# huakunyang/SummerTTS

Measured on AMD Instinct MI355X. Metric: audio samples/sec (acoustic model + vocoder, phoneme ids -> int16 PCM on host), single_speaker_fast-shaped synthetic blob, higher is better.
Workload: dtype f32 (decoder trunk convs AND the reverse flow's WaveNet convs (wn_flow.hip, one-utterance calls): fp32 operands as 2 fp16 terms = 22-23 of their 24 mantissa bits, 3 fp16 MFMA products per fp32 product, f32 accumulation -- measured error in `parity`, same tolerance as the exact-fp32 leg; batches addi

## Files before the change

include/summertts_hip.h:

```cpp
#ifndef SUMMERTTS_HIP_H_
#define SUMMERTTS_HIP_H_

#include <stdint.h>

#ifdef __cplusplus
extern "C" {
#endif

typedef struct sts_engine sts_engine;

enum {
    STS_OK = 0,
    STS_EINVAL = -1,
    STS_EMODEL = -2,
    STS_EDEVICE = -3,
    STS_ESTATE = -4
};

int sts_create(const float* blob, int64_t blob_bytes, int device, sts_engine** out);
void sts_destroy(sts_engine* e);

int sts_speaker_num(const sts_engine* e);

typedef struct sts_model_info {
// ... 100 lines not shown
#define STS_EQ_MAX_BANDS 4
#define STS_EQ_PEAK 1
#define STS_EQ_LOWSHELF 2
#define STS_EQ_HIGHSHELF 3
#define STS_EQ_HIGHPASS 4
#define STS_EQ_LOWPASS 5
typedef struct sts_eq_band { int32_t type; float freq_hz; float gain_db; float q; } sts_eq_band;
int sts_set_eq(sts_engine* e, int32_t n_bands, const sts_eq_band* bands);
int sts_get_eq(const sts_engine* e, int32_t* n_bands, sts_eq_band* bands, int32_t capacity);
int sts_eq_check(int32_t rate, int32_t n_bands, const sts_eq_band* bands);
int sts_eq_design(int32_t rate, int32_t n_bands, const sts_eq_band* bands, double* coeffs);
int sts_eq_apply(int device, const float* x, const int64_t* lengths, int32_t B, int32_t rate, int32_t n_bands,
                 const sts_eq_band* bands, float* y, int16_t* pcm);
int sts_set_record_taps(sts_engine* e, int enable);
int sts_get_tap(sts_engine* e, const char* name, float** data, int32_t* channels, int64_t* length);
int sts_get_durations(sts_engine* e, int32_t* dur, int64_t capacity);
int sts_set_conv_mode(sts_engine* e, int mode);
int sts_set_conv_math(sts_engine* e, int mode);

enum { STS_DBG_ATTN_BLOCK_MIN_WGS = 1,
       STS_DBG_TAIL_FUSED = 14 ,
       STS_DBG_UPS_ROWPH = 15 ,
       STS_DBG_CHAIN_STREAMS = 13 ,
       STS_DBG_H2P = 11 ,
       STS_DBG_H2P_TILE = 12 ,
       STS_DBG_MEMO_CLEAR = 10 ,
       STS_DBG_PCM_DIRECT = 9 ,
       STS_DBG_DDS_TAIL = 8 ,
       STS_DBG_ATTN_REG = 7 ,
       STS_DBG_LAUNCH_AHEAD = 6 ,
       STS_DBG_FLOW_FUSED = 5  };
enum { STS_DBG_STREAM_RETRY_STEP = 16, STS_DBG_STREAM_DIRECT = 17 };
enum { STS_DBG_POISON = 18 };
int sts_debug_set(sts_engine* e, int key, int value);

typedef struct sts_profile {
    float ms_text_encoder, ms_duration, ms_flow, ms_decoder, ms_total_device;
    float ms_decoder_mfma;
    int32_t decoder_mfma_launches;
    double flops_text_encoder, flops_duration, flops_flow, flops_decoder;
    double flops_decoder_mfma;
    double bytes_decoder_min;
    int64_t frames, samples, phonemes;
    double flops_decoder_mfma_executed;
    double bytes_text_encoder, bytes_duration, bytes_flow;
    float ms_sync_wait_host;
    double flops_decoder_bf16_issued;
    int64_t conv_math_fallbacks;
    int32_t conv_math_pinned;
    int32_t launch_ahead;
    int64_t launch_ahead_misses;
    float us_host_setup;
    float us_host_enqueue;
    float us_host_tail;
    int64_t poison_bytes;
} sts_profile;
int sts_set_profiling(sts_engine* e, int enable);
#define STS_ABI_VERSION 16
int sts_abi_version(void);
int sts_build_flags(void);
int sts_get_profile(const sts_engine* e, sts_profile* p);
int sts_get_profile_ex(const sts_engine* e, void* p, int64_t size_bytes);

int sts_debug_conv1d(int device, const float* x, int32_t Cin, int32_t L, const float* w, const float* bias,
                     int32_t Cout, int32_t k, int32_t pad, int32_t dil, int32_t stride_transposed,
                     int32_t depthwise, float in_slope, int32_t in_act, int mode, float** y, int32_t* Lout);
// ... 93 lines not shown
```

summertts_amd/csrc/capi.hip:

```cpp
#include <stdlib.h>
#include <string.h>

#include <algorithm>
#include <new>
#include <string>
#include <vector>

#include "engine.hpp"

using namespace sts;

struct sts_engine { Engine eng; };

static thread_local std::string g_err;
static int set_err(int code, const std::string& s) { g_err = s; return code; }

extern "C" {

const char* sts_last_error(void) { return g_err.c_str(); }
void sts_free(void* p) { free(p); }

int sts_create(const float* blob, int64_t blob_bytes, int device, sts_engine** out) {
    if (!out) return set_err(STS_EINVAL, "sts_create: null out pointer");
    *out = nullptr;
// ... 564 lines not shown
    if (!e) return set_err(STS_EINVAL, "null engine");
    if (noise_scale) *noise_scale = e->eng.noise.ns;
    if (noise_scale_w) *noise_scale_w = e->eng.noise.nsw;
    if (seed) *seed = e->eng.noise.seed;
    return STS_OK;
}
int sts_set_record_taps(sts_engine* e, int enable) { if (!e) return set_err(STS_EINVAL, "null engine"); e->eng.record_taps = enable != 0; return STS_OK; }
int sts_set_conv_math(sts_engine* e, int mode) {
    if (!e) return set_err(STS_EINVAL, "null engine");
    if (mode < 0 || mode > 3) return set_err(STS_EINVAL, "conv math: 0 = split-bf16 (default), 1 = exact fp32, 2 = split-bf16 wherever eligible, 3 = two-term fp16");
    e->eng.conv_math = mode;
    e->eng.h2_consecutive = 0; e->eng.h2_disabled = false;
    return STS_OK;
}
int sts_set_conv_mode(sts_engine* e, int mode) { if (!e) return set_err(STS_EINVAL, "null engine"); e->eng.conv_mode = mode; return STS_OK; }
int sts_debug_set(sts_engine* e, int key, int value) {
    if (!e) return set_err(STS_EINVAL, "null engine");
    switch (key) {
        case STS_DBG_ATTN_BLOCK_MIN_WGS: if (value < 1) return set_err(STS_EINVAL, "threshold must be >= 1"); e->eng.attn_block_min_wgs = value; return STS_OK;
        case STS_DBG_FLOW_FUSED: e->eng.flow_fused = value != 0; return STS_OK;
        case STS_DBG_LAUNCH_AHEAD: if (value < 0 || value > 2) return set_err(STS_EINVAL, "launch_ahead must be 0, 1 or 2"); if ((value == 2) != (e->eng.launch_ahead == 2)) { e->eng.seen_tf_.clear(); e->eng.seen_order_.clear(); } e->eng.launch_ahead = value; return STS_OK;
        case STS_DBG_H2P: e->eng.h2p = value < 0 ? 0 : (value > 4 ? 4 : value); return STS_OK;
        case STS_DBG_H2P_TILE: e->eng.h2p_tile = value; return STS_OK;
        case STS_DBG_CHAIN_STREAMS: e->eng.chain_streams_dbg = value; return STS_OK;
        case STS_DBG_TAIL_FUSED: e->eng.tail_fused = value != 0; return STS_OK;
        case STS_DBG_UPS_ROWPH: e->eng.ups_rowph = value != 0; return STS_OK;
        case STS_DBG_MEMO_CLEAR: e->eng.seen_tf_.clear(); e->eng.seen_order_.clear(); return STS_OK;
        case STS_DBG_ATTN_REG: e->eng.attn_reg = value != 0; return STS_OK;
        case STS_DBG_DDS_TAIL: e->eng.dds_tail = value != 0; return STS_OK;
        case STS_DBG_PCM_DIRECT: e->eng.pcm_direct = value != 0; return STS_OK;
        case STS_DBG_STREAM_RETRY_STEP: e->eng.stream_retry_step = value < 0 ? -1 : value; return STS_OK;
        case STS_DBG_STREAM_DIRECT: e->eng.stream_direct = value != 0; return STS_OK;
        case STS_DBG_POISON: e->eng.poison = (unsigned)value; return STS_OK;
        default: return set_err(STS_EINVAL, "unknown debug key");
    }
}
int sts_set_host_pcm(sts_engine* e, int enable) { if (!e) return set_err(STS_EINVAL, "null engine"); e->eng.host_pcm = enable != 0; return STS_OK; }
int sts_set_profiling(sts_engine* e, int enable) { if (!e) return set_err(STS_EINVAL, "null engine"); e->eng.profiling = enable == 2 ? 2 : (enable != 0 ? 1 : 0); return STS_OK; }

int sts_abi_version(void) { return STS_ABI_VERSION; }

int sts_set_output_rate(sts_engine* e, int32_t rate) {
    if (!e) return set_err(STS_EINVAL, "null engine");
    const int rc = e->eng.set_output_rate(rate);
    return rc == STS_OK ? STS_OK : set_err(rc, e->eng.error());
}
int sts_get_output_rate(const sts_engine* e) {
    if (!e) return set_err(STS_EINVAL, "null engine");
    return e->eng.out_rate;
}
int sts_resample_table(int32_t in_rate, int32_t out_rate, int32_t* P, int32_t* Q, int32_t* taps, float* table, int64_t capacity_floats) {
    ResampleDesign d;
    if (!resample_design(in_rate, out_rate, &d)) return set_err(STS_EINVAL, "rates must be integers in [8000, 48000] with P = out / gcd(in, out) <= 1024");
    const int64_t need = (int64_t)d.P * 2 * d.K;
    if (table && capacity_floats < need) return set_err(STS_EINVAL, "table capacity below P * taps floats");
    if (P) *P = d.P;
    if (Q) *Q = d.Q;
    if (taps) *taps = 2 * d.K;
    if (table) resample_table(d, in_rate, out_rate, table);
    return STS_OK;
}
int sts_set_loudness(sts_engine* e, int mode, float target_lufs, float peak_dbfs) {
    if (!e) return set_err(STS_EINVAL, "null engine");
    const int rc = e->eng.set_loudness(mode, target_lufs, peak_dbfs);
    return rc == STS_OK ? STS_OK : set_err(rc, e->eng.error());
}
// ... 631 lines not shown
```

summertts_amd/csrc/decoder.hip:

```cpp
#include "run_ctx.hpp"
#include "knobs.hpp"

#include <math.h>
#include <string.h>
#include <utility>

namespace sts {

static constexpr int MAX_HALO_H2P = 64;

int decoder_halo_frames(const Model& M) {
    double R = M.dec_type == 0 ? (M.conv_post.k - 1) / 2 : (M.conv_post.k - 1) / 2 + 12;
    const int nk = M.n_resk;
    for (int i = M.n_up - 1; i >= 0; i--) {
        double rb = 0;
        for (int j = 0; j < nk; j++) {
            const DResBlock& b = M.rb[(size_t)i * nk + j];
            double r = 0;
            for (size_t d = 0; d < b.c1.size(); d++) r += b.c1[d].dil * (b.c1[d].k - 1) / 2 + b.c2[d].dil * (b.c2[d].k - 1) / 2;
            if (r > rb) rb = r;
        }
        R += rb;
        const DConv& up = M.ups[i];
        R = ceil((R + up.k) / (double)up.stride) + 1;
// ... 48 lines not shown
    StagedMfma
};
static bool is_fused(LayerKind k) { return k == LayerKind::FusedBf3 || k == LayerKind::FusedWino || k == LayerKind::FusedDirect; }

struct LayerArgs {
    ConvGroup G1, G2;
    ResLayerGroup R;
    H2PGroup H1, H2;
    double fl, flw;
};

struct Engine::ResStage {
    Engine& e; const int i, nk, nd0; const DConv& up; const Lvl& l2; const StageBufs b;
    bool grouped = false, per_chain = false, h2p_stage = false;
    int rank[8] = {};
    const float* cur[kMaxGroup] = {};
    ResStage(Engine& e_, int i_, const Lvl& l2_, float* reg, size_t ce)
        : e(e_), i(i_), nk(e_.model.n_resk), nd0(nk > 0 ? (int)e_.model.rb[(size_t)i_ * nk].c1.size() : 0), up(e_.model.ups[i_]), l2(l2_), b{reg, ce, nk} {
        chain_rank(e.model, i, rank);
    }
    const DResBlock& rb(int j) const { return e.model.rb[(size_t)i * nk + j]; }
    hipStream_t aux(int j) const { return e.aux_[rank[j] % kAux]; }
    long fused128_tiles() const { return (long)((l2.max_len + 117) / 118) * l2.nb * nk; }
    void fork() const { (void)hipEventRecord(e.ev_fork_, e.stream); for (int k = 0; k < kAux; k++) (void)hipStreamWaitEvent(e.aux_[k], e.ev_fork_, 0); }
    void join(int n) const { for (int k = 0; k < n; k++) { (void)hipEventRecord(e.ev_join_[k], e.aux_[k]); (void)hipStreamWaitEvent(e.stream, e.ev_join_[k], 0); } }

    bool probe_grouped();
    void plan();
    bool fuse_candidate(int d) const;
    void fill_convs(int d, LayerArgs& A);
    void fill_fused(int d, ResLayerGroup& R) const;
    void fill_h2p(int d, H2PGroup& H1, H2PGroup& H2) const;
    LayerKind plan_layer(int d, LayerArgs& A) const;
    void launch(LayerKind k, int d, const LayerArgs& A) const;
    void book(LayerKind k, const LayerArgs& A);
    void run_grouped(const float** outs);
    void run_forked(const float** outs);
};

bool Engine::ResStage::probe_grouped() {
    ConvGroup G; G.n = nk;
    const double f0 = e.flops_[3], b0 = e.bytes_[3];
    for (int j = 0; j < nk; j++) G.g[j] = e.conv_args(rb(j).c1[0], b.up(), l2, b.up(), l2, ConvOpt(), nullptr);
    e.flops_[3] = f0; e.bytes_[3] = b0;
    return conv_group_eligible(G);
}

void Engine::ResStage::plan() {
    grouped = e.conv_mode == 0 && nk >= 2 && nk <= kMaxGroup;
    for (int j = 0; j < nk && grouped; j++) grouped = (int)rb(j).c1.size() == nd0;
    grouped = grouped && probe_grouped();
    if (!grouped) return;
    static const int chain_streams_env = exp_int("STS_CHAIN_STREAMS", 0);
    const int chain_streams = e.chain_streams_dbg >= 0 ? e.chain_streams_dbg : chain_streams_env;
    per_chain = ((chain_streams >> i) & 1) && nk <= kAux;
    const long h2p_tiles = (long)((l2.max_len + 127) / 128) * (up.Cout / 128) * l2.nb * nk;
    const long h2p_min = up.Cout == 128 ? 768 : 512;
    h2p_stage = e.conv_math == 3 && e.h2p && !per_chain && up.Cout % 128 == 0 && (double)l2.ld * 32.0 < 2.0e9 &&
                (e.h2p == 2 || (e.h2p == 3 && up.Cout == 128) || (e.h2p == 4 && up.Cout != 128) || h2p_tiles >= h2p_min);
    for (int j = 0; j < nk && h2p_stage; j++)
        for (int d = 0; d < nd0 && h2p_stage; d++) {
            const DConv &c1 = rb(j).c1[d], &c2 = rb(j).c2[d];
            h2p_stage = c1.wh2p && c2.wh2p && c1.Cin == up.Cout && c1.Cout == up.Cout && c2.Cin == up.Cout && c2.Cout == up.Cout &&
                        (c1.k & 1) && (c2.k & 1) && c1.dil >= 1 && c2.dil >= 1 && c1.pad == c1.dil * (c1.k - 1) / 2 && c2.pad == c2.dil * (c2.k - 1) / 2 &&
                        c1.dil * (c1.k - 1) <= MAX_HALO_H2P && c2.dil * (c2.k - 1) <= MAX_HALO_H2P && !c1.depthwise && !c2.depthwise && !c1.transposed && !c2.transposed;
        }
}

bool Engine::ResStage::fuse_candidate(int d) const {
// ... 44 lines not shown
    memset(&H1, 0, sizeof(H1)); memset(&H2, 0, sizeof(H2));
    H1.n = H2.n = nk; H1.seg = H2.seg = l2.seg; H1.B = H2.B = l2.nb; H1.max_n = H2.max_n = l2.max_len; H1.ovf = H2.ovf = e.ovf_;
    for (int j = 0; j < nk; j++) {
        const DConv &c1 = rb(j).c1[d], &c2 = rb(j).c2[d];
        float *t1 = b.t1(j), *pn = b.pn(j), *nxt = b.next(j, cur[j]);
        H2PArgs& a1 = H1.g[j];
        a1.xp = d == 0 ? (const void*)b.P0() : (const void*)pn; a1.xp_ld = l2.ld; a1.wb = c1.wh2p; a1.wscale = c1.h2_scale; a1.bias = c1.bias;
        a1.yp = t1; a1.yp_ld = l2.ld; a1.yp_slope = 0.1f;
        a1.Cin = c1.Cin; a1.Cout = c1.Cout; a1.ntap = c1.k; a1.tap_step = c1.dil; a1.tap_off = -c1.pad;
        H2PArgs& a2 = H2.g[j];
        a2.xp = t1; a2.xp_ld = l2.ld; a2.wb = c2.wh2p; a2.wscale = c2.h2_scale; a2.bias = c2.bias;
        a2.res16 = d == 0 ? b.X0() : cur[j]; a2.res_ld = l2.ld;
        if (d + 1 == nd0) { a2.y = nxt; a2.y_ld = l2.ld; }
        else { a2.y16 = nxt; a2.y16_ld = l2.ld; a2.yp = pn; a2.yp_slope = 0.1f; a2.yp_ld = l2.ld; }
        a2.Cin = c2.Cin; a2.Cout = c2.Cout; a2.ntap = c2.k; a2.tap_step = c2.dil; a2.tap_off = -c2.pad;
    }
}

LayerKind Engine::ResStage::plan_layer(int d, LayerArgs& A) const {
    const bool bf3 = e.conv_math != 1;
    if (fuse_candidate(d)) {
        fill_fused(d, A.R);
        if (resblock_layer_eligible(A.R)) {
            if (bf3 && resblock_bf3_eligible(A.R)) return LayerKind::FusedBf3;
            static const bool no_wino = exp_flag("STS_NO_WINO");
            return !no_wino && resblock_wino_eligible(A.R) ? LayerKind::FusedWino : LayerKind::FusedDirect;
        }
    }
    if (h2p_stage) { fill_h2p(d, A.H1, A.H2); return LayerKind::H2PPair; }
    if (per_chain) return bf3 ? LayerKind::StagedBf3 : LayerKind::StagedMfma;
    return bf3 && conv_bf3_group_eligible(A.G1) && conv_bf3_group_eligible(A.G2) ? LayerKind::StagedBf3 : LayerKind::StagedMfma;
}

void Engine::ResStage::launch(LayerKind k, int d, const LayerArgs& A) const {
    const hipStream_t stream = e.stream;
    static const char* gt = exp_env("STS_GROUP_TILE");
    const int gtile = gt && (int)strlen(gt) > i ? gt[i] - '0' : -1;
    if (is_fused(k)) {
        auto run = [&](const ResLayerGroup& R, hipStream_t st) {
            static const int bv = exp_int("STS_BF3_LAYER_VARIANT", -1);
            if (k == LayerKind::FusedBf3) resblock_bf3(R, st, bv);
            else if (k == LayerKind::FusedWino) resblock_wino(R, st);
            else resblock_layer(R, st);
        };
        if (!per_chain) return run(A.R, stream);
        for (int j = 0; j < nk; j++) { ResLayerGroup R1 = A.R; R1.n = 1; R1.g[0] = A.R.g[j]; run(R1, aux(j)); }
    } else if (k == LayerKind::H2PPair) {
        if (d == 0) split_planes(b.up(), l2.ld, up.Cout, l2.seg, l2.nb, l2.max_len, 0.1f, b.P0(), b.X0(), l2.ld, e.ovf_, stream);
        const int ht = e.h2p_tile < 0 ? -1 : (up.Cout == 128 ? (e.h2p_tile & 0xff) : ((e.h2p_tile >> 8) & 0xff));
        conv_h2p_group(A.H1, stream, ht == 0xff ? -1 : ht);
        conv_h2p_group(A.H2, stream, ht == 0xff ? -1 : ht);
    } else if (per_chain) {
        for (int j = 0; j < nk; j++)
            for (const ConvArgs* ca : {&A.G1.g[j], &A.G2.g[j]}) {
                if (k == LayerKind::StagedBf3 && conv_bf3_eligible(*ca)) conv_bf3(*ca, aux(j), -1);
                else if (conv_mfma_eligible(*ca)) conv_mfma(*ca, aux(j), gtile);
                else conv_generic(*ca, aux(j));
            }
    } else if (k == LayerKind::StagedBf3) {
        static const char* bgt = exp_env("STS_BF3_GROUP_TILE");
        const int bt = bgt && (int)strlen(bgt) > i ? (bgt[i] >= '0' && bgt[i] <= '9' ? bgt[i] - '0' : (bgt[i] >= 'a' && bgt[i] <= 'z' ? bgt[i] - 'a' + 10 : -1)) : -1;
        conv_bf3_group(A.G1, stream, bt);
        conv_bf3_group(A.G2, stream, bt);
    } else {
        for (const ConvGroup* G : {&A.G1, &A.G2}) {
            if (conv_group_eligible(*G)) conv_mfma_group(*G, stream, gtile);
            else for (int j = 0; j < nk; j++) { if (conv_mfma_eligible(G->g[j])) conv_mfma(G->g[j], stream, -1); else conv_generic(G->g[j], stream); }
        }
    }
}

void Engine::ResStage::book(LayerKind k, const LayerArgs& A) {
    e.mfma_flops_ += A.fl;
    if (k == LayerKind::FusedWino) e.mfma_exec_ += A.flw;
    else if (k == LayerKind::FusedDirect || k == LayerKind::StagedMfma) e.mfma_exec_ += A.fl;
    else e.bf16_exec_ += e.products() * A.fl;
    e.mfma_launches_ += is_fused(k) ? 1 : 2;
}

void Engine::ResStage::run_grouped(const float** outs) {
    LayerArgs A;
    for (int j = 0; j < nk; j++) cur[j] = b.up();
    if (per_chain) fork();
    for (int d = 0; d < nd0; d++) {
        fill_convs(d, A);
        const LayerKind k = plan_layer(d, A);
        launch(k, d, A);
        book(k, A);
        for (int j = 0; j < nk; j++) cur[j] = b.next(j, cur[j]);
    }
    if (per_chain) join(kAux);
    for (int j = 0; j < nk; j++) outs[j] = cur[j];
}

void Engine::ResStage::run_forked(const float** outs) {
    const bool forked = nk > 1 && nk <= 8;
    if (forked) fork();
    for (int j = 0; j < nk; j++) {
        if (forked) e.cur_ = aux(j);
        const float* x = b.up();
        for (size_t d = 0; d < rb(j).c1.size(); d++) {
            const auto o = resblock_opts(x);
            float* nxt = b.next(j, x);
            e.conv(rb(j).c1[d], x, l2, b.t1(j), l2, o.first);
            e.conv(rb(j).c2[d], b.t1(j), l2, nxt, l2, o.second);
            x = nxt;
        }
        outs[j] = x;
    }
    if (forked) { join(nk < kAux ? nk : kAux); e.cur_ = e.stream; }
}

int Engine::run_decode(RunCtx& c, int nw, long Wtot, int maxW, int zoff0, int wlen0) {
    RUN_ALIASES(c)
    stage_begin(3);
    const WinGeom win{nw == 1 && !no_inline_seg && wlen0 >= 0, nw, zoff0, wlen0, d_win};
    auto lvF = [&](int scale, int extra) {
        Lvl l; l.seg = win.seg(scale, extra);
        l.nb = nw; l.max_len = maxW * scale + extra;
        l.total = Wtot * scale + (long)nw * extra; l.ld = l.total;
        return l;
    };
    Lvl lz; lz.seg = win.zseg();
    lz.nb = nw; lz.max_len = maxW; lz.total = Fld; lz.ld = Fld;
    const Lvl lw1 = lvF(1, 0);
// ... 3 lines not shown
            Lvl lw; lw.seg = SegView{nullptr, nullptr, 1, 0, 0, nw}; lw.nb = 1; lw.max_len = nw; lw.total = nw; lw.ld = nw;
            if (c.mix) gather_speaker(bt.g, B, M.gin, d_win + 3 * nw, nw, bf.gwin, stream);
            else gather_speaker(M.emb_g, M.spk_num, M.gin, d_win + 3 * nw, nw, bf.gwin, stream);
            conv(M.dec_cond, bf.gwin, lw, bf.cond_win, lw, ConvOpt()); op.ubias = bf.cond_win;
        } else if (M.dec_type == 0 && ms) { conv(M.dec_cond, bt.g, lvB, bt.cond_dec, lvB, ConvOpt()); op.ubias = bt.cond_dec; }
        conv(M.conv_pre, bf.z, lz, bf.x0, lw1, op);
    }
    const float* x = bf.x0;
    int S = 1;
    Lvl lx = lw1;
    struct { const float* p[3] = {nullptr, nullptr, nullptr}; int n = 0; float* dst = nullptr; long count = 0; } mean;
    auto with_mean = [&](ConvOpt& o) { if (mean.n >= 2) { o.sum1 = mean.p[1]; o.sum2 = mean.p[2]; o.nsum = mean.n; o.sum_dst = mean.dst; o.sum_n = mean.count; } };
    static const bool no_sum_fold = exp_flag("STS_NO_SUM_FOLD");
    mark(5);
    in_mfma_region_ = true;
    for (int i = 0; i < M.n_up; i++) {
        const DConv& up = M.ups[i];
        const int S2 = S * M.up_rate[i];
        const Lvl l2 = lvF(S2, 0);
        const size_t ce = (size_t)up.Cout * l2.total;
        ResStage st(*this, i, l2, (i & 1) ? bf.regB : bf.regA, ce);
        float* bup = st.b.up();
        ConvOpt ou; ou.in_act = 1; ou.slope = 0.1f;
        {
            static const char* ut = exp_env("STS_UP_TILE");
            if (ut && (int)strlen(ut) > i && ut[i] >= '0' && ut[i] <= '7') ou.tile = ut[i] - '0';
        }
        with_mean(ou);
        conv(up, x, lx, bup, l2, ou);
        mean.n = 0;
        const int nk = st.nk;
        const float* outs[8];
        st.plan();
        if (st.grouped) st.run_grouped(outs); else st.run_forked(outs);
        if (nk == 1) x = outs[0];
        else if (nk <= 3 && !no_sum_fold) { mean.p[0] = outs[0]; mean.p[1] = outs[1]; mean.p[2] = nk > 2 ? outs[2] : nullptr; mean.n = nk; mean.dst = bup; mean.count = (long)ce; x = outs[0]; }
        else { sum_scale(bup, outs, nk, (long)ce, stream); x = bup; }
        S = S2; lx = l2;
    }
    in_mfma_region_ = false;
    mark(6);

    float* wave = c.oc.wave[OS_TAIL] ? bf.wave : nullptr;
    int16_t* const pcm = bf.pcm_nat;
    const long Ntot = Wtot * hop;
    if (M.dec_type == 0) {
        ConvOpt o; o.in_act = 1; o.slope = 1e-2f; o.epi = EPI_TANH_PCM; o.pcm = pcm; o.aux = wave;
        with_mean(o);
        conv(M.conv_post, x, lx, nullptr, lx, o);
    } else {
        const Lvl lsb = lvF(S, 1);
        ConvOpt o; o.in_act = 1; o.slope = 1e-2f; o.reflect = 1;
        with_mean(o);
        conv(M.conv_post, x, lx, bf.tailA, lsb, o);
        const int bands = M.dec_type == 2 ? 1 : 4;
        const Lvl ltm = lvF(S * 4, 0), lo = lvF(S * 16, 0);
        if (tail_fused && M.dec_type != 2 && sbC == 72 && istft_tail_fused_ok(bands, M.fir_taps, M.fir_pad)) {
            istft_tail_fused(bf.tailA, lsb.ld, lsb.seg, M.synth_fir, M.fir_taps, M.fir_pad, (float)M.subbands, M.fir_bias, wave, pcm, lo.seg, nw, ltm.max_len, stream);
        } else {
            istft_spectrum(bf.tailA, lsb.ld, sbC, bf.tailB, lsb.total, stream);
            float* tm = bf.tailC;
            istft_ola(bf.tailB, lsb.ld, bands, 18, lsb.seg, tm, ltm.ld, ltm.seg, nw, ltm.max_len, stream);
            if (M.dec_type == 2) {
                quantize_pcm(tm, pcm, Ntot, stream);
                if (wave) HIPCK(hipMemcpyAsync(wave, tm, (size_t)Ntot * 4, hipMemcpyDeviceToDevice, stream));
            } else synth_fir(tm, ltm.ld, ltm.seg, M.synth_fir, M.fir_taps, M.fir_pad, (float)M.subbands, M.fir_bias , wave, pcm, lo.seg, nw, ltm.max_len, stream);
        }
        flops_[3] += 2.0 * (double)Ntot * (16.0 * 4 + 4 * 18 * 4 / 4.0);
// ... 100 lines not shown
```

summertts_amd/csrc/engine.hpp:

```cpp
#pragma once
#include <hip/hip_runtime.h>

#include <deque>
#include <map>
#include <unordered_map>
#include <string>
#include <vector>

#include "../../include/summertts_hip.h"
#include "kernels.hpp"
#include "model.hpp"

namespace sts {

struct Arena {
    char* base = nullptr; size_t cap = 0, used = 0; bool measuring = false;
    void* alloc(size_t bytes) {
        size_t a = (used + 255) & ~(size_t)255;
        used = a + bytes;
        if (measuring) return nullptr;
        return base + a;
    }
    template <typename T> T* get(size_t count) { return (T*)alloc(count * sizeof(T)); }
};
// ... 82 lines not shown
    std::vector<int64_t> last_join_start;
    int run_joined(int B, const int32_t* const* ids, const int32_t* n, const int32_t* sid, const float* ls, const sts_join* join);
    int join_offsets(int64_t* start, int64_t capacity);
    std::vector<int32_t> last_n;
    int phoneme_offsets(int64_t* start, int64_t capacity);
    bool record_taps = false; int profiling = 0;
    int conv_mode = 0;
    int conv_math = 3;
    long h2_fallbacks = 0;
    int h2_consecutive = 0; bool h2_disabled = false;
    double products() const { return conv_math == 3 ? 3.0 : 6.0; }
    int pcm_direct = 1;
    int dds_tail = 1;
    int attn_reg = 1;
    int attn_block_min_wgs = 96;
    int launch_ahead = 1;
    long ahead_misses = 0;
    static constexpr size_t kMemoEntries = 1024;
    std::unordered_map<unsigned long long, long> seen_tf_; std::deque<unsigned long long> seen_order_;
    bool polite_wait = false;
    struct WaitEst { double us = 0.0; long phonemes = 0; };
    WaitEst wait_est_[2][24];
    void nap_before_wait(int which, long phonemes);
    void note_wait(int which, long phonemes, double waited_us, bool was_ready_at_wake);
    int final_sync(long phonemes);
    int ups_rowph = 1;
    int tail_fused = 1;
    int chain_streams_dbg = -1;
    int h2p = 1;
    int h2p_tile = -1;
    int flow_fused = 1;
    int stream_retry_step = -1;
    int stream_direct = 0;
    unsigned poison = 0;
    int64_t poison_bytes_ = 0;
    hipStream_t stream = nullptr;

private:
    int fail(int code, const std::string& msg) { err_ = msg; return code; }
    bool ensure(Arena& a, size_t bytes);
    bool ensure_pinned(size_t bytes);
    void poison_arena(const Arena& a);
    void poison_host16(void* p, size_t samples);
    void poison_host32(void* p, size_t words);
    ConvArgs conv_args(const DConv& c, const float* x, const Lvl& lin, float* y, const Lvl& lout, const ConvOpt& o, double* flops);
    void conv(const DConv& c, const float* x, const Lvl& lin, float* y, const Lvl& lout, const ConvOpt& o);
    void ln(const DLn& l, const float* a, const float* b, const float* res, float* y, const Lvl& lv, int pre_relu, int post_gelu, int nb = 1, long b_stride = 0);
    int pick_kslices(const DConv& c, const Lvl& lout) const;
    struct SplineTail { const DConv* proj; float filter_sqrt; const float* r0; const float* r1; float* o0; float* o1; };
    float* dds(const DDds& d, float* h, float* t1, float* t2, const Lvl& lv, const DConv* pre = nullptr, const float* pre_in = nullptr,
               const float* pre_res = nullptr, const SplineTail* tail = nullptr, bool* tail_done = nullptr);
    int run_any_math(int B, const int32_t* const* ids, const int32_t* n, const int32_t* sid, const float* ls, const StreamSpec* ss);
    struct RunCtx;
    struct ResStage;
    int run_setup(RunCtx& c);
    int run_text_encoder(RunCtx& c);
    int run_durations(RunCtx& c);
    int run_frame_workspace(RunCtx& c);
    int run_flow(RunCtx& c);
    int run_decode(RunCtx& c, int nw, long Wtot, int maxW, int zoff0, int wlen0);
    int decode_end(RunCtx& c, const float* wave, const WinGeom& win, long Wtot, int maxW);
    int wait_frame_counts(RunCtx& c);
    int plan_output(RunCtx& c);
    int frame_geometry(RunCtx& c);
    int run_output(RunCtx& c);
    int run_stream_steps(RunCtx& c);
// ... 36 lines not shown
```

summertts_amd/csrc/kernels.hpp:

```cpp
#pragma once
#include <hip/hip_runtime.h>
#include <stdint.h>

#include <vector>

#include "../../include/summertts_hip.h"

namespace sts {

struct SegView {
    const int* off;
    const int* len;
    int scale;
    int extra;
    int ioff, ilen;
};

enum Epilogue : int {
    EPI_STORE = 0,
    EPI_RESADD = 1,
    EPI_SUB = 3,
    EPI_GATE = 4,
    EPI_RESSKIP = 5,
    EPI_TANH_PCM = 6,
// ... 121 lines not shown
bool conv_mfma_eligible(const ConvArgs& a);
void conv_mfma(const ConvArgs& a, hipStream_t st, int tile = -1);
constexpr int kMaxGroup = 4;
struct ConvGroup { ConvArgs g[kMaxGroup]; int n; };
struct ResLayerArgs {
    const float* x; float* y;
    const float *w1, *b1, *w2, *b2;
    int k1, dil1, k2;
    const float *wu1, *wu2;
    const void *wb1, *wb2;
    float ws1, ws2;
};
struct ResLayerGroup {
    ResLayerArgs g[kMaxGroup];
    int n, C; long ld; float slope;
    SegView seg; int B; int max_n;
    int math; unsigned* ovf;
};
bool resblock_layer_eligible(const ResLayerGroup& G);
void resblock_layer(const ResLayerGroup& G, hipStream_t st);
bool resblock_wino_eligible(const ResLayerGroup& G);
void resblock_wino(const ResLayerGroup& G, hipStream_t st);
bool conv_group_eligible(const ConvGroup& G);
bool conv_bf3_eligible(const ConvArgs& a);
bool conv_bf3_takes_sum(const ConvArgs& a);
bool conv_cout1_takes(const ConvArgs& a);
void conv_bf3(const ConvArgs& a, hipStream_t st, int tile = -1);
long conv_bf3_blocks(const ConvArgs& a);
bool conv_bf3_group_eligible(const ConvGroup& G);
void conv_bf3_group(const ConvGroup& G, hipStream_t st, int tile = -1);
size_t bf3_pack(const float* wp, int nphase, int ntap, int Cin_pad, int Cout_pad, void* dst, bool perm_k = false, int math = 0, float* wscale = nullptr);
bool resblock_bf3_eligible(const ResLayerGroup& G);
void resblock_bf3(const ResLayerGroup& G, hipStream_t st, int variant = -1);
void conv_mfma_group(const ConvGroup& G, hipStream_t st, int tile = -1);

struct H2PArgs {
    const void* xp; long xp_ld;
    const void* wb; float wscale;
    const float* bias;
    const float* res16; long res_ld;
    float* y; long y_ld;
    float* y16; long y16_ld;
    void* yp; long yp_ld; float yp_slope;
    int Cin, Cout, ntap, tap_step, tap_off;
};
struct H2PGroup { H2PArgs g[kMaxGroup]; int n; SegView seg; int B, max_n; unsigned* ovf; };
bool conv_h2p_group_eligible(const H2PGroup& G);
void conv_h2p_group(const H2PGroup& G, hipStream_t st, int tile = -1);
struct H2WArgs {
    const float* x16; long x_ld;
    const void* wu; float wscale;
    const float* bias;
    const float* res16; long res_ld;
    float* y16; long y16_ld;
    float* y; long y_ld;
    float in_slope, out_slope;
    int C, k, dil;
};
struct H2WGroup { H2WArgs g[kMaxGroup]; int n; SegView seg; int B, max_n; unsigned* ovf; };
bool conv_h2w_group_eligible(const H2WGroup& G);
void conv_h2w_group(const H2WGroup& G, hipStream_t st);
int h2w_transform_weights(const float* wp, int k, int Cin, int Cout, float* dst);
void to_x16(const float* x, long x_ld, int C, long n, float* x16, long out_ld, hipStream_t st);
void split_planes(const float* x, long x_ld, int C, const SegView& seg, int nb, long max_n, float slope, void* planes, float* x16, long out_ld,
                  unsigned* ovf, hipStream_t st);
void conv_generic(const ConvArgs& a, hipStream_t st);
// ... 167 lines not shown
```

summertts_amd/csrc/resblock_bf3.hip:

```cpp
#include "conv_bf3_dev.hpp"

namespace sts {

#ifdef STS_TILE_TRACE
int tile_trace_bind_resblock(long long* buf, unsigned capacity_records) { return tile_trace_bind(buf, capacity_records); }
#endif

#ifndef STS_RB_WAVES
#define STS_RB_WAVES 3
#endif
#ifndef STS_RB_ADEPTH
#define STS_RB_ADEPTH 2
#endif
#ifndef STS_RB_EXP
#define STS_RB_EXP 0
#endif
#ifndef STS_RB_RES_LATE
#define STS_RB_RES_LATE 0
#endif
template <int MW, int WM, int NW, int WN, int MATH = 0>
__global__ __launch_bounds__(64 * WM * WN) __attribute__((amdgpu_waves_per_eu(MW == 1 ? STS_RB_WAVES : 2, MW == 1 ? STS_RB_WAVES : 2))) void resblock_bf3_kernel(ResLayerGroup G, int nx, int wst, int interleave) {
    constexpr int C = 32 * MW * WM, NCH = C / 16, NRT = C / 32, NWAVE = WM * WN, P1 = 32 * NW * WN;
    constexpr int NPB = MATH ? 2 : 3;
    constexpr int NPA = MATH ? 2 : 3;
// ... 237 lines not shown
    TT_STAMP(4);
    {
        static_for<0, MW>([&](auto ic) {
            constexpr int i = decltype(ic)::value;
            static_for<0, NW>([&](auto qc) {
                constexpr int q = decltype(qc)::value;
                const int col = wn * NW * 32 + q * 32 + m4;
                const int pos = n0 + col;
                const bool any = col < NT && pos < len, full = col + 3 < NT && pos + 3 < len;
#pragma unroll
                for (int g = 0; g < 4; g++) {
                    float w[4] = {acc[i][q][4 * g], acc[i][q][4 * g + 1], acc[i][q][4 * g + 2], acc[i][q][4 * g + 3]};
                    quad_transpose(w, l31);
                    if (any) {
                        f32x4u o;
#pragma unroll
                        for (int e = 0; e < 4; e++) o[e] = (MATH ? w[e] * a.ws2 : w[e]) + b2v[i][g] + xres[i][q][g][e];
                        float* yp = a.y + (size_t)(mbase + i * 32 + 8 * g + 4 * half + lane4) * G.ld + base + pos;
                        if (full) *(f32x4u*)yp = o;
                        else { for (int e = 0; e < 4; e++) if (col + e < NT && pos + e < len) yp[e] = o[e]; }
                    }
                }
            });
        });
    }
    if constexpr (MATH == 1) { if (amax > kH2Limit && G.ovf) *G.ovf = 1u; }
#ifdef STS_TILE_TRACE
    asm volatile("s_waitcnt vmcnt(0)" ::: "memory");
    TT_STAMP(5);
    TT_CLOSE();
#endif
}

bool resblock_bf3_eligible(const ResLayerGroup& G) {
    if (G.n < 1 || G.n > kMaxGroup || (G.C != 32 && G.C != 64 && G.C != 128) || G.max_n <= 0 || G.B <= 0) return false;
    if ((double)G.ld * 64.0 >= 4.0e9) return false;
    for (int i = 0; i < G.n; i++) {
        const ResLayerArgs& a = G.g[i];
        if (!a.wb1 || !a.wb2 || !(a.k1 & 1) || !(a.k2 & 1) || a.k1 < 1 || a.k2 < 1) return false;
        if (a.dil1 < 1 || a.dil1 * (a.k1 - 1) > MAX_HALO || a.k2 - 1 > 32) return false;
        if (a.x == a.y) return false;
    }
    return true;
}

template <int MW, int WM, int NW, int WN>
static void launch_resblock_bf3(const ResLayerGroup& G, hipStream_t st) {
    constexpr int C = 32 * MW * WM, P1 = 32 * NW * WN;
    int nx = 0, halo = 0;
    for (int i = 0; i < G.n; i++) {
        const int NT = P1 - (G.g[i].k2 - 1);
        const int n = (G.max_n + NT - 1) / NT;
        if (n > nx) nx = n;
        const int h = G.g[i].dil1 * (G.g[i].k1 - 1);
        if (h > halo) halo = h;
    }
    const int wst = (P1 + halo + 31) / 32 * 32;
    const size_t pb = G.math == 1 ? 4 : 6;
    const size_t stage = (size_t)C * wst * pb, park = (size_t)C * P1 * pb + 1024;
    const size_t lds = stage > park ? stage : park;
    static const int il = exp_int("STS_BF3_INTERLEAVE", 0);
    if (G.math == 1)
        hipLaunchKernelGGL((resblock_bf3_kernel<MW, WM, NW, WN, 1>), dim3(mapped_grid(nx, 1, G.B * G.n)), dim3(64 * WM * WN), lds, st, G, nx, wst, (il >> 1) & 1);
    else
        hipLaunchKernelGGL((resblock_bf3_kernel<MW, WM, NW, WN>), dim3(mapped_grid(nx, 1, G.B * G.n)), dim3(64 * WM * WN), lds, st, G, nx, wst, (il >> 1) & 1);
}

void resblock_bf3(const ResLayerGroup& Gin, hipStream_t st, int variant) {
    ResLayerGroup G = Gin;
    for (int i = 1; i < G.n; i++)
        for (int j = i; j > 0 && G.g[j].k1 + G.g[j].k2 > G.g[j - 1].k1 + G.g[j - 1].k2; j--) {
            ResLayerArgs t = G.g[j]; G.g[j] = G.g[j - 1]; G.g[j - 1] = t;
        }
    if (G.C == 128) {
        if (variant == 1) launch_resblock_bf3<2, 2, 2, 2>(G, st); else launch_resblock_bf3<1, 4, 2, 2>(G, st);
    } else if (G.C == 64) {
        if (variant == 1) launch_resblock_bf3<2, 1, 2, 2>(G, st); else launch_resblock_bf3<1, 2, 2, 2>(G, st);
    } else {
        if (variant == 1) launch_resblock_bf3<1, 1, 2, 2>(G, st); else launch_resblock_bf3<1, 1, 2, 4>(G, st);
    }
}

}
```

summertts_amd/engine.py:

```python
from __future__ import annotations

import ctypes as C
import os
import subprocess
from typing import Dict, List, Optional, Sequence

import numpy as np

_HERE = os.path.dirname(os.path.abspath(__file__))
LIB_PATH = os.environ.get("SUMMERTTS_HIP_LIB") or os.path.join(_HERE, "lib", "libsummertts_hip.so")
CSRC = os.path.join(_HERE, "csrc")


def build_library(verbose: bool = False) -> str:
    subprocess.run(["make", "-C", CSRC, "-j8"], check=True, stdout=None if verbose else subprocess.DEVNULL)
    return LIB_PATH


class ModelInfo(C.Structure):
    _fields_ = [("is_multi_speaker", C.c_int32), ("lang_type", C.c_int32), ("dur_pred_type", C.c_int32),
                ("dec_type", C.c_int32), ("vocab", C.c_int32), ("hidden", C.c_int32), ("inter_channels", C.c_int32),
                ("speaker_num", C.c_int32), ("gin_channels", C.c_int32), ("samples_per_frame", C.c_int32),
                ("sample_rate", C.c_int32), ("blob_floats_consumed", C.c_int64)]

# ... 817 lines not shown
        n, arr = _eq_bands(bands)
        _check(self.lib, self.lib.sts_set_eq(self.h, n, arr))

    def get_eq(self):
        n = C.c_int32()
        arr = (EqBand * EQ_MAX_BANDS)()
        _check(self.lib, self.lib.sts_get_eq(self.h, C.byref(n), arr, EQ_MAX_BANDS))
        return [(int(arr[i].type), float(arr[i].freq_hz), float(arr[i].gain_db), float(arr[i].q)) for i in range(n.value)]

    def limiter_mode(self):
        m, g, c, l = C.c_int(), C.c_float(), C.c_float(), C.c_float()
        _check(self.lib, self.lib.sts_get_limiter_mode(self.h, C.byref(m), C.byref(g), C.byref(c), C.byref(l)))
        return m.value, g.value, c.value, l.value

    def limiter(self) -> np.ndarray:
        n = self.lib.sts_get_limiter(self.h, None, 0)
        if n < 0:
            _check(self.lib, n)
        out = np.zeros(n, LIMITER_DTYPE)
        if n:
            rc = self.lib.sts_get_limiter(self.h, out.ctypes.data, n)
            if rc < 0:
                _check(self.lib, rc)
        return out

    def set_conv_math(self, mode):
        m = {"bf16x3": 0, "f32": 1, "bf16x3_all": 2, "f16x2": 3}.get(mode, mode)
        _check(self.lib, self.lib.sts_set_conv_math(self.h, int(m)))

    def set_conv_mode(self, mode: int):
        _check(self.lib, self.lib.sts_set_conv_mode(self.h, mode))

    def debug_set(self, key: str, value: int):
        _check(self.lib, self.lib.sts_debug_set(self.h, {"attn_block_min_wgs": 1, "flow_fused": 5, "launch_ahead": 6, "attn_reg": 7, "dds_tail": 8, "pcm_direct": 9, "memo_clear": 10, "h2p": 11, "h2p_tile": 12, "chain_streams": 13, "tail_fused": 14, "ups_rowph": 15, "stream_retry_step": 16, "stream_direct": 17, "poison": 18}[key], int(value)))

    def set_profiling(self, on):
        _check(self.lib, self.lib.sts_set_profiling(self.h, 2 if on == 2 else (1 if on else 0)))

    def profile(self) -> dict:
        p = Profile()
        _check(self.lib, self.lib.sts_get_profile_ex(self.h, C.byref(p), C.sizeof(p)))
        return p.as_dict()

    def tap(self, name: str) -> np.ndarray:
        ptr = C.POINTER(C.c_float)()
        ch, ln = C.c_int32(), C.c_int64()
        _check(self.lib, self.lib.sts_get_tap(self.h, name.encode(), C.byref(ptr), C.byref(ch), C.byref(ln)))
        a = np.ctypeslib.as_array(ptr, shape=(ch.value, ln.value)).copy()
        self.lib.sts_free(ptr)
        return a

    def durations(self, total_phonemes: int) -> np.ndarray:
        d = np.zeros(total_phonemes, np.int32)
        _check(self.lib, self.lib.sts_get_durations(self.h, d.ctypes.data, d.size))
        return d

    def close(self):
        if getattr(self, "h", None) is not None and self.h:
            self.lib.sts_destroy(self.h)
            self.h = None

    def __del__(self):
        try:
            self.close()
        except Exception:
            pass

# ... 394 lines not shown
```

Before: 67.26 million.

## Fuse last resblock layer across parallel chains with in-kernel mean reduction

Adds a join kernel for the final dilation layer of the grouped resblock stage. One workgroup runs every kernel-size chain for its tile in sequence, keeps the running residual sum in registers, and writes the averaged result straight to the upsample buffer. This removes the separate per-chain outputs and the later mean/sum_scale pass, along with their memory traffic. In exchange, each workgroup serialises the chains, so there are fewer workgroups (grid over B rather than B*n), and the kernel only covers C=32 or 64 with 2-3 chains.

```diff
diff --git a/include/summertts_hip.h b/include/summertts_hip.h
--- a/include/summertts_hip.h
+++ b/include/summertts_hip.h
@@ -156,6 +156,7 @@
        STS_DBG_FLOW_FUSED = 5  };
 enum { STS_DBG_STREAM_RETRY_STEP = 16, STS_DBG_STREAM_DIRECT = 17 };
 enum { STS_DBG_POISON = 18 };
+enum { STS_DBG_CHAIN_JOIN = 19 };
 int sts_debug_set(sts_engine* e, int key, int value);
 
 typedef struct sts_profile {
diff --git a/summertts_amd/csrc/capi.hip b/summertts_amd/csrc/capi.hip
--- a/summertts_amd/csrc/capi.hip
+++ b/summertts_amd/csrc/capi.hip
@@ -620,6 +620,7 @@
         case STS_DBG_STREAM_RETRY_STEP: e->eng.stream_retry_step = value < 0 ? -1 : value; return STS_OK;
         case STS_DBG_STREAM_DIRECT: e->eng.stream_direct = value != 0; return STS_OK;
         case STS_DBG_POISON: e->eng.poison = (unsigned)value; return STS_OK;
+        case STS_DBG_CHAIN_JOIN: if (value < 0 || value > 2) return set_err(STS_EINVAL, "chain_join must be 0, 1 or 2"); e->eng.chain_join = value; return STS_OK;
         default: return set_err(STS_EINVAL, "unknown debug key");
     }
 }
diff --git a/summertts_amd/csrc/decoder.hip b/summertts_amd/csrc/decoder.hip
--- a/summertts_amd/csrc/decoder.hip
+++ b/summertts_amd/csrc/decoder.hip
@@ -104,9 +104,10 @@
     void fill_fused(int d, ResLayerGroup& R) const;
     void fill_h2p(int d, H2PGroup& H1, H2PGroup& H2) const;
     LayerKind plan_layer(int d, LayerArgs& A) const;
-    void launch(LayerKind k, int d, const LayerArgs& A) const;
+    bool plan_join(LayerKind k, int d, LayerArgs& A) const;
+    void launch(LayerKind k, int d, const LayerArgs& A, bool joined) const;
     void book(LayerKind k, const LayerArgs& A);
-    void run_grouped(const float** outs);
+    int run_grouped(const float** outs);
     void run_forked(const float** outs);
 };
 
@@ -217,8 +218,18 @@
     return bf3 && conv_bf3_group_eligible(A.G1) && conv_bf3_group_eligible(A.G2) ? LayerKind::StagedBf3 : LayerKind::StagedMfma;
 }
 
-void Engine::ResStage::launch(LayerKind k, int d, const LayerArgs& A) const {
+bool Engine::ResStage::plan_join(LayerKind k, int d, LayerArgs& A) const {
+    if (!e.chain_join || per_chain || nd0 < 2 || d + 1 != nd0 || k != LayerKind::FusedBf3) return false;
+    ResLayerGroup R = A.R;
+    for (int j = 0; j < nk; j++) R.g[j].y = b.up();
+    if (!resblock_bf3_join_eligible(R)) return false;
+    A.R = R;
+    return true;
+}
+
+void Engine::ResStage::launch(LayerKind k, int d, const LayerArgs& A, bool joined) const {
     const hipStream_t stream = e.stream;
+    if (joined) return resblock_bf3_join(A.R, stream);
     static const char* gt = exp_env("STS_GROUP_TILE");
     const int gtile = gt && (int)strlen(gt) > i ? gt[i] - '0' : -1;
     if (is_fused(k)) {
@@ -263,19 +274,23 @@
     e.mfma_launches_ += is_fused(k) ? 1 : 2;
 }
 
-void Engine::ResStage::run_grouped(const float** outs) {
+int Engine::ResStage::run_grouped(const float** outs) {
     LayerArgs A;
+    bool joined = false;
     for (int j = 0; j < nk; j++) cur[j] = b.up();
     if (per_chain) fork();
     for (int d = 0; d < nd0; d++) {
         fill_convs(d, A);
         const LayerKind k = plan_layer(d, A);
-        launch(k, d, A);
+        joined = plan_join(k, d, A);
+        launch(k, d, A, joined);
         book(k, A);
         for (int j = 0; j < nk; j++) cur[j] = b.next(j, cur[j]);
     }
     if (per_chain) join(kAux);
+    if (joined) { outs[0] = b.up(); return 1; }
     for (int j = 0; j < nk; j++) outs[j] = cur[j];
+    return nk;
 }
 
 void Engine::ResStage::run_forked(const float** outs) {
@@ -345,8 +360,9 @@
         const int nk = st.nk;
         const float* outs[8];
         st.plan();
-        if (st.grouped) st.run_grouped(outs); else st.run_forked(outs);
-        if (nk == 1) x = outs[0];
+        int nout = nk;
+        if (st.grouped) nout = st.run_grouped(outs); else st.run_forked(outs);
+        if (nout == 1) x = outs[0];
         else if (nk <= 3 && !no_sum_fold) { mean.p[0] = outs[0]; mean.p[1] = outs[1]; mean.p[2] = nk > 2 ? outs[2] : nullptr; mean.n = nk; mean.dst = bup; mean.count = (long)ce; x = outs[0]; }
         else { sum_scale(bup, outs, nk, (long)ce, stream); x = bup; }
         S = S2; lx = l2;
diff --git a/summertts_amd/csrc/engine.hpp b/summertts_amd/csrc/engine.hpp
--- a/summertts_amd/csrc/engine.hpp
+++ b/summertts_amd/csrc/engine.hpp
@@ -138,6 +138,7 @@
     int flow_fused = 1;
     int stream_retry_step = -1;
     int stream_direct = 0;
+    int chain_join = 1;
     unsigned poison = 0;
     int64_t poison_bytes_ = 0;
     hipStream_t stream = nullptr;
diff --git a/summertts_amd/csrc/kernels.hpp b/summertts_amd/csrc/kernels.hpp
--- a/summertts_amd/csrc/kernels.hpp
+++ b/summertts_amd/csrc/kernels.hpp
@@ -177,6 +177,8 @@
 size_t bf3_pack(const float* wp, int nphase, int ntap, int Cin_pad, int Cout_pad, void* dst, bool perm_k = false, int math = 0, float* wscale = nullptr);
 bool resblock_bf3_eligible(const ResLayerGroup& G);
 void resblock_bf3(const ResLayerGroup& G, hipStream_t st, int variant = -1);
+bool resblock_bf3_join_eligible(const ResLayerGroup& G);
+void resblock_bf3_join(const ResLayerGroup& G, hipStream_t st);
 void conv_mfma_group(const ConvGroup& G, hipStream_t st, int tile = -1);
 
 struct H2PArgs {
diff --git a/summertts_amd/csrc/resblock_bf3.hip b/summertts_amd/csrc/resblock_bf3.hip
--- a/summertts_amd/csrc/resblock_bf3.hip
+++ b/summertts_amd/csrc/resblock_bf3.hip
@@ -293,6 +293,271 @@
 #endif
 }
 
+template <int WM, int NW, int WN, int MATH>
+__global__ __launch_bounds__(64 * WM * WN) __attribute__((amdgpu_waves_per_eu(STS_RB_WAVES, STS_RB_WAVES))) void resblock_bf3_join_kernel(ResLayerGroup G, int nx, int wst) {
+    constexpr int C = 32 * WM, NCH = C / 16, NRT = C / 32, NWAVE = WM * WN, P1 = 32 * NW * WN;
+    constexpr int NPB = MATH ? 2 : 3;
+    constexpr int NPA = MATH ? 2 : 3;
+    constexpr unsigned ABLK = NPA * 1024u;
+    constexpr int PLANE2 = P1 * 32, CHUNK2 = NPB * PLANE2;
+    constexpr int MAXSLOT = (P1 + MAX_HALO) / 32;
+    constexpr int ITEMS = (NCH * MAXSLOT + NWAVE - 1) / NWAVE;
+    constexpr int AD = 2;
+    extern __shared__ __attribute__((aligned(16))) unsigned char smem3[];
+    const TileId t = map_tile(nx, 1, G.B);
+    if (!t.valid) return;
+    const int tbx = t.bx, b = t.bz;
+    const ResLayerArgs* const ka = (const ResLayerArgs*)__builtin_amdgcn_kernarg_segment_ptr();
+    int h2max = 0;
+    for (int j = 0; j < G.n; j++) { const int h = (ka[j].k2 - 1) / 2; h2max = h > h2max ? h : h2max; }
+    const int NT = P1 - 2 * h2max;
+    const int len = seg_len(G.seg, b);
+    const int n0 = tbx * NT;
+    if (n0 >= len) return;
+    const size_t base = (size_t)seg_start(G.seg, b);
+    const int plane1 = wst * 32, chunk1 = NPB * plane1;
+    const unsigned ld4 = (unsigned)G.ld * 4u;
+    float amax = 0.f;
+    u32x4 fa[AD][1][NPA], fb[2][NW][NPB];
+    f32x4u S[NW][4];
+    f32x16 acc[1][NW];
+    auto mfmas = [&](u32x4 (&ac)[1][NPA], u32x4 (&bc)[NW][NPB]) { step_mfmas<MATH, 1, NW, NPA, NPB>(acc, ac, bc); };
+
+    for (int jm = 0; jm < G.n; jm++) {
+        int tid = threadIdx.x;
+        asm volatile("" : "+v"(tid));
+        const int lane = tid & 63, wave = tid >> 6;
+        const int swave = __builtin_amdgcn_readfirstlane(wave);
+        const int wn = wave % WN, wm = wave / WN;
+        const int mbase = wm * 32;
+        const int l31 = lane & 31, half = lane >> 5;
+        const int lane4 = l31 & 3, m4 = (l31 >> 2) * 4;
+        const unsigned a_voff = (unsigned)lane * 16u + (unsigned)(mbase >> 5) * ABLK;
+        auto load_a = [&](const rsrc_t& wrs, int s, u32x4 (&dst)[1][NPA]) {
+            const unsigned sb = (unsigned)s * ((unsigned)NRT * ABLK);
+#pragma unroll
+            for (int pl = 0; pl < NPA; pl++)
+                dst[0][pl] = __builtin_bit_cast(u32x4, __builtin_amdgcn_raw_buffer_load_b128(wrs, (int)a_voff, (int)(sb + (unsigned)(pl * 1024)), 0));
+        };
+        const ResLayerArgs& a = ka[jm];
+        const int d = a.dil1;
+        const int h1 = d * (a.k1 - 1) / 2, h2 = (a.k2 - 1) / 2;
+        const int W1 = P1 + 2 * h1, nslot = (W1 + 31) >> 5;
+        const int w0 = n0 - h2 - h1;
+        const int nsteps1 = NCH * a.k1, nsteps2 = NCH * a.k2;
+        const rsrc_t wrs1 = make_rsrc(a.wb1, (unsigned)(nsteps1 * NRT) * ABLK), wrs2 = make_rsrc(a.wb2, (unsigned)(nsteps2 * NRT) * ABLK);
+        load_a(wrs1, 0, fa[0]);
+        if (jm > 0) __syncthreads();
+
+        {
+            float xr[ITEMS][8];
+            int lw[ITEMS];
+            const int nitem = NCH * nslot;
+#pragma unroll
+            for (int i = 0; i < ITEMS; i++) {
+                const int it = swave + i * NWAVE;
+                const int c = it / nslot, sl = it - c * nslot;
+                const int col = sl * 32 + l31, pos = w0 + col;
+                const bool v = col < W1 && pos >= 0 && pos < len;
+                const unsigned voff = v ? (unsigned)half * 8u * ld4 + (unsigned)pos * 4u : kOOB;
+                lw[i] = c * chunk1 + col * 32 + ((half ^ ((col >> 3) & 1)) << 4);
+#pragma unroll
+                for (int e = 0; e < 8; e++) xr[i][e] = 0.f;
+                if (it < nitem) {
+                    const rsrc_t rs = make_rsrc(a.x + (size_t)c * CK * G.ld + base, (unsigned)((15ul * G.ld + len) * 4ul));
+#pragma unroll
+                    for (int e = 0; e < 8; e++)
+                        xr[i][e] = __builtin_bit_cast(float, __builtin_amdgcn_raw_buffer_load_b32(rs, (int)voff, (int)((unsigned)e * ld4), 0));
+                }
+            }
+#pragma unroll
+            for (int i = 0; i < ITEMS; i++) {
+                const int it = swave + i * NWAVE;
+                if (it < nitem) {
+                    float v[8];
+#pragma unroll
+                    for (int e = 0; e < 8; e++) v[e] = xr[i][e] < 0.f ? xr[i][e] * G.slope : xr[i][e];
+                    if constexpr (MATH == 0) {
+                        u32x4 ph, pm, pl;
+                        split8(v, ph, pm, pl);
+                        *(u32x4*)(smem3 + lw[i]) = ph;
+                        *(u32x4*)(smem3 + plane1 + lw[i]) = pm;
+                        *(u32x4*)(smem3 + 2 * plane1 + lw[i]) = pl;
+                    } else {
+                        u32x4 ph, pl;
+                        split8h(v, ph, pl, amax);
+                        *(u32x4*)(smem3 + lw[i]) = ph;
+                        *(u32x4*)(smem3 + plane1 + lw[i]) = pl;
+                    }
+                }
+            }
+        }
+
+        float b2v[4];
+        f32x4u xin[NW][4];
+#pragma unroll
+        for (int g = 0; g < 4; g++) {
+            const int row = mbase + 8 * g + 4 * half + lane4;
+            b2v[g] = a.b2 ? a.b2[row] : 0.f;
+#pragma unroll
+            for (int q = 0; q < NW; q++) {
+                const int col = wn * NW * 32 + q * 32 + m4;
+                const int pos = n0 + col;
+                xin[q][g] = f32x4u{0.f, 0.f, 0.f, 0.f};
+                if (col < NT && pos < len) {
+                    const float* xp = a.x + (size_t)row * G.ld + base + pos;
+                    if (col + 3 < NT && pos + 3 < len) xin[q][g] = *(const f32x4u*)xp;
+                    else { for (int e = 0; e < 4; e++) if (col + e < NT && pos + e < len) xin[q][g][e] = xp[e]; }
+                }
+            }
+        }
+#pragma unroll
+        for (int q = 0; q < NW; q++)
+#pragma unroll
+            for (int g = 0; g < 4; g++) {
+                if (jm == 0) S[q][g] = xin[q][g];
+                else S[q][g] = S[q][g] + xin[q][g];
+#pragma unroll
+                for (int e = 0; e < 4; e++) asm volatile("" : "+v"(S[q][g][e]));
+            }
+#pragma unroll
+        for (int q = 0; q < NW; q++)
+#pragma unroll
+            for (int r = 0; r < 16; r++) acc[0][q][r] = 0.f;
+        __syncthreads();
+
+        {
+            const int p0 = wn * NW * 32 + l31;
+            auto load_b = [&](int c, int j, u32x4 (&dst)[NW][NPB]) {
+                const int p = p0 + j * d;
+                const unsigned char* sb = smem3 + c * chunk1 + p * 32 + ((half ^ ((p >> 3) & 1)) << 4);
+#pragma unroll
+                for (int q = 0; q < NW; q++)
+#pragma unroll
+                    for (int pl = 0; pl < NPB; pl++) dst[q][pl] = *(const u32x4*)(sb + pl * plane1 + q * 1024);
+            };
+            int sj = 0, sc = 0;
+            load_b(0, 0, fb[0]);
+            for (int s = 0; s < nsteps1; s += 2 * AD)
+                static_for<0, 2 * AD>([&](auto uc) {
+                    constexpr int u = decltype(uc)::value;
+                    if (s + u < nsteps1) {
+                        int nj = sj + 1, nc = sc;
+                        if (nj == a.k1) { nj = 0; nc = sc + 1; }
+                        load_a(wrs1, s + u + AD - 1, fa[(u + AD - 1) % AD]);
+                        load_b(nc < NCH ? nc : 0, nj, fb[(u + 1) % 2]);
+                        __builtin_amdgcn_sched_barrier(0);
+                        mfmas(fa[u % AD], fb[u % 2]);
+                        sj = nj; sc = nc;
+                    }
+                });
+        }
+        load_a(wrs2, 0, fa[0]);
+        __syncthreads();
+        {
+            float b1v[16];
+#pragma unroll
+            for (int r = 0; r < 16; r++) b1v[r] = 0.f;
+            if (a.b1) {
+#pragma unroll
+                for (int r = 0; r < 16; r++) b1v[r] = a.b1[mbase + (r >> 3) * 16 + 8 * ((r & 7) >> 2) + 4 * half + (r & 3)];
+            }
+            static_for<0, NW>([&](auto qc) {
+                constexpr int q = decltype(qc)::value;
+                const int col = wn * NW * 32 + q * 32 + l31;
+                const int pos = n0 - h2 + col;
+                const bool inside = pos >= 0 && pos < len;
+                static_for<0, 2>([&](auto hc) {
+                    constexpr int hh = decltype(hc)::value;
+                    const int cc = (mbase >> 4) + hh;
+                    float v[8];
+#pragma unroll
+                    for (int e = 0; e < 8; e++) {
+                        float t1 = (MATH ? acc[0][q][hh * 8 + e] * a.ws1 : acc[0][q][hh * 8 + e]) + b1v[hh * 8 + e];
+                        t1 = t1 < 0.f ? t1 * G.slope : t1;
+                        v[e] = inside ? t1 : 0.f;
+                        acc[0][q][hh * 8 + e] = 0.f;
+                    }
+                    unsigned char* dst = smem3 + cc * CHUNK2 + col * 32 + ((half ^ ((col >> 3) & 1)) << 4);
+                    if constexpr (MATH == 0) {
+                        u32x4 ph, pm, pl;
+                        split8(v, ph, pm, pl);
+                        *(u32x4*)(dst) = ph;
+                        *(u32x4*)(dst + PLANE2) = pm;
+                        *(u32x4*)(dst + 2 * PLANE2) = pl;
+                    } else {
+                        u32x4 ph, pl;
+                        split8h(v, ph, pl, amax);
+                        *(u32x4*)(dst) = ph;
+                        *(u32x4*)(dst + PLANE2) = pl;
+                    }
+                });
+            });
+        }
+        __syncthreads();
+
+        {
+            const int p0 = wn * NW * 32 + l31;
+            auto load_b = [&](int c, int j, u32x4 (&dst)[NW][NPB]) {
+                const int p = p0 + j;
+                const unsigned char* sb = smem3 + c * CHUNK2 + p * 32 + ((half ^ ((p >> 3) & 1)) << 4);
+#pragma unroll
+                for (int q = 0; q < NW; q++)
+#pragma unroll
+                    for (int pl = 0; pl < NPB; pl++) dst[q][pl] = *(const u32x4*)(sb + pl * PLANE2 + q * 1024);
+            };
+            int sj = 0, sc = 0;
+            load_b(0, 0, fb[0]);
+            for (int s = 0; s < nsteps2; s += 2 * AD)
+                static_for<0, 2 * AD>([&](auto uc) {
+                    constexpr int u = decltype(uc)::value;
+                    if (s + u < nsteps2) {
+                        int nj = sj + 1, nc = sc;
+                        if (nj == a.k2) { nj = 0; nc = sc + 1; }
+                        load_a(wrs2, s + u + AD - 1, fa[(u + AD - 1) % AD]);
+                        load_b(nc < NCH ? nc : 0, nj, fb[(u + 1) % 2]);
+                        __builtin_amdgcn_sched_barrier(0);
+                        mfmas(fa[u % AD], fb[u % 2]);
+                        sj = nj; sc = nc;
+                    }
+                });
+        }
+        static_for<0, NW>([&](auto qc) {
+            constexpr int q = decltype(qc)::value;
+#pragma unroll
+            for (int g = 0; g < 4; g++) {
+                float w[4] = {acc[0][q][4 * g], acc[0][q][4 * g + 1], acc[0][q][4 * g + 2], acc[0][q][4 * g + 3]};
+                quad_transpose(w, l31);
+#pragma unroll
+                for (int e = 0; e < 4; e++) S[q][g][e] = (MATH ? w[e] * a.ws2 : w[e]) + b2v[g] + S[q][g][e];
+            }
+        });
+    }
+    {
+        const int tid = threadIdx.x, lane = tid & 63, wave = tid >> 6;
+        const int wn = wave % WN, mbase = (wave / WN) * 32;
+        const int l31 = lane & 31, half = lane >> 5, lane4 = l31 & 3, m4 = (l31 >> 2) * 4;
+        const float div = (float)G.n;
+#pragma unroll
+        for (int q = 0; q < NW; q++) {
+            const int col = wn * NW * 32 + q * 32 + m4;
+            const int pos = n0 + col;
+            if (!(col < NT && pos < len)) continue;
+            const bool full = col + 3 < NT && pos + 3 < len;
+#pragma unroll
+            for (int g = 0; g < 4; g++) {
+                f32x4u o;
+#pragma unroll
+                for (int e = 0; e < 4; e++) o[e] = S[q][g][e] / div;
+                float* yp = ka[0].y + (size_t)(mbase + 8 * g + 4 * half + lane4) * G.ld + base + pos;
+                if (full) *(f32x4u*)yp = o;
+                else { for (int e = 0; e < 4; e++) if (col + e < NT && pos + e < len) yp[e] = o[e]; }
+            }
+        }
+    }
+    if constexpr (MATH == 1) { if (amax > kH2Limit && G.ovf) *G.ovf = 1u; }
+}
+
 bool resblock_bf3_eligible(const ResLayerGroup& G) {
     if (G.n < 1 || G.n > kMaxGroup || (G.C != 32 && G.C != 64 && G.C != 128) || G.max_n <= 0 || G.B <= 0) return false;
     if ((double)G.ld * 64.0 >= 4.0e9) return false;
@@ -327,6 +592,40 @@
         hipLaunchKernelGGL((resblock_bf3_kernel<MW, WM, NW, WN>), dim3(mapped_grid(nx, 1, G.B * G.n)), dim3(64 * WM * WN), lds, st, G, nx, wst, (il >> 1) & 1);
 }
 
+bool resblock_bf3_join_eligible(const ResLayerGroup& G) {
+    if (!resblock_bf3_eligible(G) || (G.C != 32 && G.C != 64) || G.n < 2 || G.n > 3 || (G.math != 0 && G.math != 1)) return false;
+    for (int i = 0; i < G.n; i++) {
+        if (G.g[i].y != G.g[0].y) return false;
+        for (int j = 0; j < G.n; j++) if (G.g[j].x == G.g[i].y) return false;
+    }
+    return true;
+}
+
+template <int WM, int WN>
+static void launch_resblock_bf3_join(const ResLayerGroup& G, hipStream_t st) {
+    constexpr int C = 32 * WM, P1 = 64 * WN;
+    int k2max = 1, halo = 0;
+    for (int i = 0; i < G.n; i++) {
+        if (G.g[i].k2 > k2max) k2max = G.g[i].k2;
+        const int h = G.g[i].dil1 * (G.g[i].k1 - 1);
+        if (h > halo) halo = h;
+    }
+    const int NT = P1 - (k2max - 1);
+    const int nx = (G.max_n + NT - 1) / NT;
+    const int wst = (P1 + halo + 31) / 32 * 32;
+    const size_t pb = G.math == 1 ? 4 : 6;
+    const size_t stage = (size_t)C * wst * pb, park = (size_t)C * P1 * pb + 1024;
+    const size_t lds = stage > park ? stage : park;
+    if (G.math == 1)
+        hipLaunchKernelGGL((resblock_bf3_join_kernel<WM, 2, WN, 1>), dim3(mapped_grid(nx, 1, G.B)), dim3(64 * WM * WN), lds, st, G, nx, wst);
+    else
+        hipLaunchKernelGGL((resblock_bf3_join_kernel<WM, 2, WN, 0>), dim3(mapped_grid(nx, 1, G.B)), dim3(64 * WM * WN), lds, st, G, nx, wst);
+}
+
+void resblock_bf3_join(const ResLayerGroup& G, hipStream_t st) {
+    if (G.C == 64) launch_resblock_bf3_join<2, 2>(G, st); else launch_resblock_bf3_join<1, 4>(G, st);
+}
+
 void resblock_bf3(const ResLayerGroup& Gin, hipStream_t st, int variant) {
     ResLayerGroup G = Gin;
     for (int i = 1; i < G.n; i++)
diff --git a/summertts_amd/engine.py b/summertts_amd/engine.py
--- a/summertts_amd/engine.py
+++ b/summertts_amd/engine.py
@@ -873,7 +873,7 @@
         _check(self.lib, self.lib.sts_set_conv_mode(self.h, mode))
 
     def debug_set(self, key: str, value: int):
-        _check(self.lib, self.lib.sts_debug_set(self.h, {"attn_block_min_wgs": 1, "flow_fused": 5, "launch_ahead": 6, "attn_reg": 7, "dds_tail": 8, "pcm_direct": 9, "memo_clear": 10, "h2p": 11, "h2p_tile": 12, "chain_streams": 13, "tail_fused": 14, "ups_rowph": 15, "stream_retry_step": 16, "stream_direct": 17, "poison": 18}[key], int(value)))
+        _check(self.lib, self.lib.sts_debug_set(self.h, {"attn_block_min_wgs": 1, "flow_fused": 5, "launch_ahead": 6, "attn_reg": 7, "dds_tail": 8, "pcm_direct": 9, "memo_clear": 10, "h2p": 11, "h2p_tile": 12, "chain_streams": 13, "tail_fused": 14, "ups_rowph": 15, "stream_retry_step": 16, "stream_direct": 17, "poison": 18, "chain_join": 19}[key], int(value)))
 
     def set_profiling(self, on):
         _check(self.lib, self.lib.sts_set_profiling(self.h, 2 if on == 2 else (1 if on else 0)))
```

New measurement: 67.72 million (median of 4 runs). No clear change (+0.7%).
